# agustinus/emqx

Hardware: AMD Instinct MI355X
Metric: publishes matched/sec (node) at 1M wildcard subs; p99 batch match latency (higher is better)
Workload: dtype u32; 1 GPU; C2: 1M wildcard filters depth<=7, 10M-publish batch per GPU; filters=1000000, publishes_per_gpu=10000000, mode=replicated, parallelism=replicated trie x1, batches split per GPU, batches_in_flight=1

## Files before the change

### emqx_amd/csrc/tm_batch.cpp

```cpp
#include "tm_engine_impl.hpp"

int tm_engine::ensure_slow_scratch(tm_batch* b) {
    int rc;
    if (!b->s_waves) {
        uint32_t w = b->n < 65536 ? 64u : std::min<uint32_t>(TM_SLOW_WAVES_MAX, b->n / 32);
        b->s_waves = w;
    }
    const size_t q = (size_t)b->s_waves * b->s_qcap, o = (size_t)b->s_waves * b->s_ocap;
    if ((rc = b->gen.d_sqpar.reserve(q))) return rc;
    if ((rc = b->gen.d_sqpw.reserve(q))) return rc;
    if ((rc = b->gen.d_sqmeta.reserve(q))) return rc;
    if ((rc = b->gen.d_sqkey.reserve(q))) return rc;
    if ((rc = b->gen.d_sofid.reserve(o))) return rc;
    if ((rc = b->gen.d_sokey.reserve(o))) return rc;
    return TM_OK;
}

void tm_engine::tokenize_range(const TokView& v, uint32_t lo, uint32_t hi, std::vector<uint32_t>& slow_out) const {
    std::vector<TWord> ws;
    for (uint32_t t = lo; t < hi; ++t) {
        const uint8_t* p = v.bytes + v.offs[t];
        const size_t len = v.offs[t + 1] - v.offs[t];
        split_words(p, len, ws);
        uint32_t* out = v.words + v.toff[t];
// ... 867 lines not shown
    HIP_OK(launch_scan(b->scan_args, S, b->dcsr.d_total.p));
    HIP_OK(launch_finalize(b->scan_args, S, checked));
    HIP_OK(hipEventRecord(b->dcsr.evc1.e, S));
    HIP_OK(hipMemcpyAsync(b->dcsr.h_total.p, b->dcsr.d_total.p, 4, hipMemcpyDeviceToHost, S));
    HIP_OK(hipStreamSynchronize(S));
    if (b->dcsr.h_total.p[0] != b->total) {
        snprintf(last_error(), 512, "inconsistent CSR: scanned %u entries, kernel count %llu", b->dcsr.h_total.p[0],
                 (unsigned long long)b->total);
        return TM_EIO;
    }
    float ms = 0;
    (void)hipEventElapsedTime(&ms, b->dcsr.evc0.e, b->dcsr.evc1.e);
    b->st.ms_csr = ms;
    b->dense = true;
    return TM_OK;
}

int tm_engine::check_ctrl(const uint32_t* ctrl, const unsigned long long* stats, uint32_t* err, uint64_t* need,
               uint64_t* staged_out) {
    *err = ctrl[CTRL_ERR];
    uint64_t staged = 0, top = 0;
    for (uint32_t g = 0; g < TICKET_GROUPS; ++g) {
        const uint64_t t = xg_top_read(ctrl, g);
        staged += t;
        top = std::max(top, t);
    }
    *need = top * TICKET_GROUPS;
    if (staged_out) *staged_out = staged;
    const uint64_t nmatch = stats[ST_MATCHES];
    if ((*err & ERR_CSR_RANGE) || staged > result_limit || nmatch > result_limit) {
        snprintf(last_error(), 512, "batch result too large: %llu staged / %llu matched > limit %llu",
                 (unsigned long long)staged, (unsigned long long)nmatch, (unsigned long long)result_limit);
        return TM_EOVERFLOW;
    }
    return TM_OK;
}

int tm_engine::grow_for(tm_batch* b, uint32_t err, uint64_t need, uint64_t staged) {
    if (err & ERR_STAGING) {
        const uint64_t limit = std::min<uint64_t>(MAX_RESULT, result_limit + 1024);
        if (!b->one_region && need + need / 4 + 1024 > limit && staged <= result_limit) b->one_region = true;
        if (b->one_region) need = staged;
        int rc = b->walk.d_sfids.reserve(std::min<uint64_t>(need + need / 4 + 1024, limit));
        if (rc) return rc;
    }
    if (err & ERR_SLOW_SCRATCH) {
        b->s_qcap *= 4;
        b->s_ocap *= 4;
    }
    return TM_OK;
}

void tm_engine::fill_stats(tm_batch* b) {
    float ms_match = 0, ms_total = 0, ms_tok = 0, ms_dd = 0, ms_x = 0;
    (void)hipEventElapsedTime(&ms_match, b->walk.ev0.e, b->walk.ev1.e);
    (void)hipEventElapsedTime(&ms_total, b->walk.ev0.e, b->walk.ev2.e);
    if (b->tok_timed) (void)hipEventElapsedTime(&ms_tok, b->tok.evt.e, b->walk.ev0.e);
    if (b->dedup_timed) (void)hipEventElapsedTime(&ms_dd, b->dd.evd.e, b->tok_timed ? b->tok.evt.e : b->walk.ev0.e);
    if (b->dedup_dev && !b->graphed) (void)hipEventElapsedTime(&ms_x, b->dd.evx0.e, b->dd.evx1.e);
    b->st.ms_tokenize = ms_tok;
    b->st.ms_dedup = ms_dd;
    b->st.ms_expand = ms_x;
    b->st.publishes = b->dedup ? b->n_pub : b->n;
    float ms_q = 0;
    (void)hipEventElapsedTime(&ms_q, b->walk.evq.e,
                              b->dedup_timed ? b->dd.evd.e : b->tok_timed ? b->tok.evt.e : b->walk.ev0.e);
    b->st.ms_queue = ms_q;
    b->st.ms_csr = 0;
    b->st.topics = b->n;
    b->st.visits = b->walk.h_stats[ST_VISITS];
    b->st.hash_hits = b->walk.h_stats[ST_HASH];
    b->st.words = b->walk.h_stats[ST_WORDS];
    b->st.matches = b->walk.h_stats[ST_MATCHES];
    b->st.slow_topics = b->walk.h_stats[ST_SLOW];
    b->st.probes = b->walk.h_stats[ST_PROBES];
    b->st.iterations = b->walk.h_stats[ST_ITERS];
    b->st.overflow_tiles = b->walk.h_ctrl[CTRL_NOVF];
    b->st.ms_match = ms_match;
    b->st.ms_total = ms_total;
    b->total = b->st.matches;
    b->st.delivered = b->dedup_dev ? b->walk.h_stats[ST_DELIVERED] : b->st.matches;
#if TM_PHASE_CYCLES
    fprintf(stderr, "tm_phase_cycles prologue=%llu loop=%llu readback=%llu sort=%llu ms_match=%.4f\n",
            b->h_stats[ST_PHASE + 0], b->h_stats[ST_PHASE + 1], b->h_stats[ST_PHASE + 2], b->h_stats[ST_PHASE + 3],
            ms_match);
#endif
}

int tm_engine::wait(tm_batch* b, bool drained, uint32_t* relaunched) {
    if (!b->launched) return TM_EINVAL;
    const hipStream_t S = st(b);
    if (!b->csr) {
        int rc = launch(b, true);
        if (rc) return rc;
        drained = false;
    }
    for (int attempt = 0;; ++attempt) {
        if (!drained || attempt) {
            if (b->end_recorded) HIP_OK(hipEventSynchronize(b->walk.ev_end.e));
            else HIP_OK(hipStreamSynchronize(S));
        }
        if (attempt && relaunched) ++*relaunched;
        if (b->dedup_dev) {
            b->n = b->walk.h_ctrl[CTRL_NROWS];
            b->scan_args.n = b->n;
        }
        if (b->check_tokens && b->n && b->tok.h_bad.p[1]) {
            snprintf(last_error(), 512, "token batch failed the device check (word offsets or flags)");
            return TM_EINVAL;
        }
        const uint32_t* h_dbg = b->rep->tab.h_dbg.p;
        if (checked && h_dbg[0]) {
            snprintf(last_error(), 512, "bounds check %u failed: index %u bound %u (count %u, extra %u)",
                     h_dbg[0], h_dbg[1], h_dbg[2], h_dbg[3], h_dbg[4]);
            return TM_EIO;
        }
        uint32_t err;
        uint64_t need, staged;
        int rc = check_ctrl(b->walk.h_ctrl, b->walk.h_stats, &err, &need, &staged);
        if (rc) return rc;
        if (!err) break;
        if (attempt >= 6) {
            snprintf(last_error(), 512, "capacity misses did not settle after %d relaunches (err %#x, %llu staged)",
                     attempt, err, (unsigned long long)staged);
            return TM_EOVERFLOW;
        }
        if ((rc = grow_for(b, err, need, staged))) return rc;
        if ((rc = launch(b))) return rc;
    }
    fill_stats(b);
    b->done = true;
    if (b->dedup_dev) b->dtab_dirty = false;
    b->dense = b->dense_enq && !b->oneshot && b->total <= b->dense_cap;
    if (b->dense) {
        float ms = 0;
        (void)hipEventElapsedTime(&ms, b->dcsr.evc0.e, b->dcsr.evc1.e);
        b->st.ms_csr = ms;
    }
    return TM_OK;
}

int tm_engine::result(tm_batch* b, tm_result* out) {
    if (!b->done) return TM_EINVAL;
    int rc;
    if ((rc = ensure_dense(b))) return rc;
    const hipStream_t S = st(b);
    const uint64_t total = b->total;
    if (total > b->dcsr.d_ids.cap) {
        snprintf(last_error(), 512, "inconsistent CSR: kernel count %llu, capacity %zu",
                 (unsigned long long)total, b->dcsr.d_ids.cap);
        return TM_EIO;
    }
    if ((rc = b->dcsr.h_rowoff.reserve((size_t)b->n + 1))) return rc;
    if ((rc = b->dcsr.h_ids.reserve(std::max<uint64_t>(total, 1)))) return rc;
    HIP_OK(hipMemcpyAsync(b->dcsr.h_rowoff.p, b->dcsr.d_rowoff.p, ((size_t)b->n + 1) * 4, hipMemcpyDeviceToHost, S));
    if (total) HIP_OK(hipMemcpyAsync(b->dcsr.h_ids.p, b->dcsr.d_ids.p, total * 4, hipMemcpyDeviceToHost, S));
    HIP_OK(hipStreamSynchronize(S));
    if (b->dcsr.h_rowoff.p[b->n] != total) {
        snprintf(last_error(), 512, "inconsistent CSR: row offsets end at %u, kernel count %llu",
                 b->dcsr.h_rowoff.p[b->n], (unsigned long long)total);
        return TM_EIO;
    }
    out->n_topics = b->n;
    out->n_matches = total;
    out->row_offsets = b->dcsr.h_rowoff.p;
    out->filter_ids = b->dcsr.h_ids.p;
    return TM_OK;
// ... 88 lines not shown
```

### emqx_amd/csrc/tm_kernels.hip

```cpp
#include <algorithm>
#include <cstddef>
#include <cstdlib>
#include "tm_internal.hpp"

namespace etm {

constexpr int TILE = 64;
constexpr int WCAP = 512;
#ifndef TM_WPE384
#define TM_WPE384 4
#endif

constexpr uint32_t M_LVL_SHIFT = 6;
constexpr uint32_t M_LVL_MASK = 0xF;
constexpr uint32_t M_PLUS = 1u << 10;
constexpr uint32_t M_SKIPE = 1u << 11;
constexpr uint32_t M_DSTART = 1u << 12;
static_assert(FAST_MAX_DEPTH <= (int)M_LVL_MASK, "level field too narrow");
constexpr uint32_t M_DISP_SHIFT = 13;
constexpr uint32_t M_DISP_MASK = 0x3F;
constexpr uint32_t Q_FOUND = ~((1u << LSIG_BITS) - 1u);
constexpr uint32_t Q_TAIL = 0xFFFFFFFFu;

__device__ __forceinline__ uint32_t dig_L(uint32_t c) { return (0x4432u >> (4 * c)) & 0xF; }
// ... 89 lines not shown
    if (x.np == 0) { x.pk0 = key; x.pf0 = fl; } else { x.pk1 = key; x.pf1 = fl; }
    x.np++;
}

__device__ __forceinline__ void expand(const Node& s, uint32_t lc, uint32_t d, uint32_t flags,
                                       uint64_t key, uint32_t w_here, uint32_t w_prev, Expand& x) {
    x.ne = 0; x.np = 0;
    if (lc == d) {
        if (!(flags & M_SKIPE) && s.term != NONE) {
            uint64_t k = key;
            if ((w_prev >> WID_BITS) == C_EMPTY && lc - 1 <= FAST_MAX_DEPTH) {
                const int sp = key_shift(lc - 1);
                if (((k >> sp) & 7) == 4) k = (k & ~(7ull << sp)) | (1ull << sp);
            }
            add_e(x, s.term, k);
        }
        if (s.hterm != NONE) add_e(x, s.hterm, put_digit(key, lc, 2));
        return;
    }
    const uint32_t cls = w_here >> WID_BITS, id = w_here & WID_MASK;
    if (s.hterm != NONE) add_e(x, s.hterm, put_digit(key, lc, dig_H(cls)));
    if (id == W_HASH) {
        if (s.flags & NF_HASH) add_p(x, put_digit(key, lc, dig_L(cls)), (lc + 1 == d) ? M_SKIPE : 0u);
    } else if (id != W_UNKNOWN && id != W_PLUS) {
        add_p(x, put_digit(key, lc, dig_L(cls)), 0u);
    }
    if (s.flags & NF_PLUS) add_p(x, put_digit(key, lc, dig_P(cls)), M_PLUS);
}

__device__ __forceinline__ void expand_root(const RootRec& r, bool dollar, uint32_t d, uint32_t w0, Expand& x) {
    x.ne = 0; x.np = 0;
    const uint32_t cls = w0 >> WID_BITS, id = w0 & WID_MASK;
    if (!dollar && r.hterm != NONE) add_e(x, r.hterm, (uint64_t)dig_H(cls) << 61);
    if (id == W_HASH) {
        if (!dollar && (r.flags & NF_HASH)) add_p(x, (uint64_t)dig_L(cls) << 61, (d == 1) ? M_SKIPE : 0u);
    } else if (id != W_UNKNOWN && id != W_PLUS) {
        add_p(x, (uint64_t)dig_L(cls) << 61, dollar ? M_DSTART : 0u);
    }
    if (!dollar && (r.flags & NF_PLUS)) add_p(x, (uint64_t)dig_P(cls) << 61, M_PLUS);
}

template <int QC>
struct alignas(16) TileLds {
    static constexpr int QCAP = QC;
    uint4 q[QC];
    uint32_t words[WCAP];
    uint32_t toff[TILE];
    uint32_t depth[TILE];
    uint32_t cnt[TILE];
    uint32_t list[TILE];
    static constexpr uint32_t STAGE = (QC * 16 + WCAP * 4) / 8;
};

__device__ __forceinline__ uint4 q_pack(uint64_t key, uint32_t meta, uint32_t parent, uint32_t pw) {
    return uint4{(uint32_t)key | meta, (uint32_t)(key >> 32), parent, pw};
}

static_assert(offsetof(TileLds<512>, words) + sizeof(uint32_t) * WCAP == TileLds<512>::STAGE * 8,
              "staging area must be contiguous");
static_assert(offsetof(TileLds<384>, words) + sizeof(uint32_t) * WCAP == TileLds<384>::STAGE * 8,
              "staging area must be contiguous");

__device__ __forceinline__ uint32_t xor_lane32(uint32_t v, uint32_t j) {
    const uint32_t lane = threadIdx.x & 63;
    switch (j) {
    case 1: return (uint32_t)__builtin_amdgcn_mov_dpp((int)v, 0xB1, 0xF, 0xF, false);
    case 2: return (uint32_t)__builtin_amdgcn_mov_dpp((int)v, 0x4E, 0xF, 0xF, false);
    case 4: return (uint32_t)__builtin_amdgcn_mov_dpp(__builtin_amdgcn_mov_dpp((int)v, 0x141, 0xF, 0xF, false), 0x1B, 0xF,
                                                      0xF, false);
    case 8: return (uint32_t)__builtin_amdgcn_mov_dpp((int)v, 0x128, 0xF, 0xF, false);
    case 16: {
        const auto p = __builtin_amdgcn_permlane16_swap(v, v, false, false);
        return (lane & 16) ? p[0] : p[1];
    }
    default: {
        const auto p = __builtin_amdgcn_permlane32_swap(v, v, false, false);
        return (lane & 32) ? p[0] : p[1];
    }
    }
}

__device__ __forceinline__ unsigned long long xor_lane64(unsigned long long v, uint32_t j) {
    return ((unsigned long long)xor_lane32((uint32_t)(v >> 32), j) << 32) | xor_lane32((uint32_t)v, j);
}

enum : int { PH_PROLOGUE = 0, PH_LOOP = 1, PH_READBACK = 2, PH_SORT = 3 };
struct PhaseClk {
#if TM_PHASE_CYCLES
    unsigned long long sum[PHASE_N] = {0, 0, 0, 0}, t0 = 0;
    __device__ __forceinline__ void start() { t0 = __builtin_readcyclecounter(); }
    __device__ __forceinline__ void lap(int p) {
        const unsigned long long now = __builtin_readcyclecounter();
        sum[p] += now - t0;
        t0 = now;
    }
#else
    __device__ __forceinline__ void start() {}
    __device__ __forceinline__ void lap(int) {}
#endif
};

__device__ __forceinline__ uint32_t xor_lane32_bc(uint32_t v, uint32_t j) {
    const int x = (int)v;
    switch (j) {
    case 1: return (uint32_t)__builtin_amdgcn_update_dpp(0, x, 0xB1, 0xF, 0xF, true);
    case 2: return (uint32_t)__builtin_amdgcn_update_dpp(0, x, 0x4E, 0xF, 0xF, true);
    case 4: return (uint32_t)__builtin_amdgcn_update_dpp(0, __builtin_amdgcn_update_dpp(0, x, 0x141, 0xF, 0xF, true),
                                                         0x1B, 0xF, 0xF, true);
    default: return (uint32_t)__builtin_amdgcn_update_dpp(0, x, 0x128, 0xF, 0xF, true);
    }
}

#ifndef TM_TAGGED_SORT
#define TM_TAGGED_SORT 1
#endif
constexpr uint64_t keep_lo_mask(uint32_t W, uint32_t kk, uint32_t j) {
    uint64_t m = 0;
    for (uint32_t l = 0; l < 64; ++l) {
        const uint32_t e = l & (W - 1);
        if (((e & j) == 0) == ((e & kk) == 0)) m |= 1ull << l;
    }
    return m;
}

template <uint32_t W, uint32_t KK, uint32_t J>
__device__ __forceinline__ uint32_t tag_stage(uint32_t k) {
    constexpr uint64_t M = keep_lo_mask(W, KK, J);
    uint32_t lo, hi;
    if constexpr (J >= 16) {
        const auto p = J == 16 ? __builtin_amdgcn_permlane16_swap(k, k, false, false)
                               : __builtin_amdgcn_permlane32_swap(k, k, false, false);
        lo = min(p[0], p[1]);
        hi = max(p[0], p[1]);
    } else {
        const uint32_t other = xor_lane32_bc(k, J);
        lo = min(k, other);
        hi = max(k, other);
    }
    return __builtin_amdgcn_inverse_ballot_w64(M) ? lo : hi;
}
template <uint32_t W, uint32_t KK, uint32_t J>
__device__ __forceinline__ uint32_t tag_merge(uint32_t k) {
    k = tag_stage<W, KK, J>(k);
    if constexpr (J > 1) k = tag_merge<W, KK, J / 2>(k);
    return k;
}
template <uint32_t W, uint32_t KK = 2>
__device__ __forceinline__ uint32_t tag_sort(uint32_t k) {
    k = tag_merge<W, KK, KK / 2>(k);
    if constexpr (KK < W) k = tag_sort<W, KK * 2>(k);
    return k;
}

template <bool CK, class LT>
__device__ __forceinline__ void sort_classes(const MatchArgs& a, LT& L, bool keep, uint32_t c, uint32_t pos,
                                             uint32_t dst, uint32_t free) {
    constexpr uint32_t STAGE = LT::STAGE;
    const uint32_t lane = threadIdx.x;
    const unsigned long long* stg = reinterpret_cast<const unsigned long long*>(L.q);
    if (keep && c == 1) a.sfids[CK_(dst, a.sfids_cap, 40)] = (uint32_t)(stg[CK_(pos, STAGE, 41)] & ~KEY_MASK);
#pragma unroll
    for (uint32_t W = 2; W <= 64; W <<= 1) {
        const bool mine = keep && c > W / 2 && c <= W;
        const uint64_t m = __ballot(mine);
        if (!m) continue;
        const uint32_t nrows = __popcll(m);
        if (mine) L.list[prefix_count(m)] = lane;
        __syncthreads();
        const uint32_t e = lane & (W - 1);
        const uint32_t STEP = 64 / W;
        for (uint32_t g = 0; g < nrows; g += STEP) {
            const uint32_t r = g + lane / W;
            const bool rv = r < nrows;
            const uint32_t owner = rv ? L.list[r] : 0u;
            const uint32_t cr = __shfl(c, owner, 64);
            const uint32_t pr = __shfl(pos, owner, 64);
            const uint32_t dr = __shfl(dst, owner, 64);
            if (TM_TAGGED_SORT && (W >> free) <= 1) {
                const uint32_t* stg32 = reinterpret_cast<const uint32_t*>(L.q);
                uint32_t k32 = 0xFFFFFFFFu;
                if (rv && e < cr) k32 = stg32[2 * CK_(pr + e, STAGE, 42) + 1] | e;
                switch (W) {
                case 2: k32 = tag_sort<2>(k32); break;
                case 4: k32 = tag_sort<4>(k32); break;
                case 8: k32 = tag_sort<8>(k32); break;
                case 16: k32 = tag_sort<16>(k32); break;
                case 32: k32 = tag_sort<32>(k32); break;
                default: k32 = tag_sort<64>(k32); break;
                }
                if (rv && e < cr)
                    a.sfids[CK_((uint64_t)dr + e, a.sfids_cap, 44)] =
                        stg32[2 * CK_(pr + (k32 & (W - 1)), STAGE, 43)] & (uint32_t)~KEY_MASK;
                continue;
            }
            unsigned long long key = ~0ull;
            if (rv && e < cr) key = stg[CK_(pr + e, STAGE, 42)];
#pragma unroll
            for (uint32_t kk = 2; kk <= W; kk <<= 1) {
#pragma unroll
                for (uint32_t j = kk >> 1; j > 0; j >>= 1) {
                    const unsigned long long other = xor_lane64(key, j);
                    const bool up = (e & kk) == 0;
                    const bool lower = (e & j) == 0;
                    const unsigned long long lo = key < other ? key : other;
                    const unsigned long long hi = key < other ? other : key;
                    key = (lower == up) ? lo : hi;
                }
            }
            if (rv && e < cr) a.sfids[CK_((uint64_t)dr + e, a.sfids_cap, 44)] = (uint32_t)(key & ~KEY_MASK);
        }
        __syncthreads();
    }
    {
        const bool mine = keep && c > 64;
        uint64_t m = __ballot(mine);
        while (m) {
            const uint32_t owner = (uint32_t)__builtin_ctzll(m);
            m &= m - 1;
            const uint32_t cr = __shfl(c, owner, 64);
            const uint32_t pr = __shfl(pos, owner, 64);
            const uint32_t dr = __shfl(dst, owner, 64);
            unsigned long long k0 = ~0ull, k1 = ~0ull;
            if (lane < cr) k0 = stg[CK_(pr + lane, STAGE, 45)];
            if (lane + 64 < cr) k1 = stg[CK_(pr + lane + 64, STAGE, 46)];
            uint32_t r0 = 0, r1 = 0;
            for (uint32_t j = 0; j < 64; ++j) {
                const unsigned long long kj = __shfl(k0, j, 64);
                r0 += kj < k0 ? 1u : 0u;
                r1 += kj < k1 ? 1u : 0u;
            }
            for (uint32_t j = 64; j < cr; ++j) {
                const unsigned long long kj = __shfl(k1, j - 64, 64);
                r0 += kj < k0 ? 1u : 0u;
                r1 += kj < k1 ? 1u : 0u;
            }
            if (lane < cr) a.sfids[CK_((uint64_t)dr + r0, a.sfids_cap, 47)] = (uint32_t)(k0 & ~KEY_MASK);
            if (lane + 64 < cr) a.sfids[CK_((uint64_t)dr + r1, a.sfids_cap, 48)] = (uint32_t)(k1 & ~KEY_MASK);
        }
    }
}

#ifndef TM_LOG_U
#define TM_LOG_U 12
#endif
template <bool CK, class LT>
__device__ __forceinline__ void sort_rows_log(const MatchArgs& a, LT& L, bool keep, uint32_t c, uint32_t dst,
                                              unsigned long long* wlog, uint8_t* wlane, uint32_t lcount,
                                              PhaseClk& pc) {
    constexpr uint32_t STAGE = LT::STAGE;
    const uint32_t lane = threadIdx.x;
    unsigned long long* stg = reinterpret_cast<unsigned long long*>(L.q);
    const uint32_t cw = keep ? c : 0u;
    uint32_t incl = cw;
    for (int o = 1; o < 64; o <<= 1) {
        const uint32_t u = __shfl_up(incl, o, 64);
        if (lane >= (uint32_t)o) incl += u;
    }
    const uint32_t pos = incl - cw;
    uint32_t rs = 0;
    while (rs < a.tile_topics) {
        const uint32_t p0 = __builtin_amdgcn_readlane(pos, rs);
        const uint64_t beyond = __ballot(lane >= rs && pos + cw - p0 > STAGE);
        const uint32_t re = beyond ? (uint32_t)__builtin_ctzll(beyond) : a.tile_topics;
        const bool in_chunk = keep && lane >= rs && lane < re;
        L.depth[lane] = in_chunk ? pos - p0 : NONE;
        L.toff[lane] = 0;
        __syncthreads();
        uint32_t kor = 0;
        for (uint32_t k0 = 0; k0 < lcount; k0 += 64 * TM_LOG_U) {
            unsigned long long e[TM_LOG_U];
            uint32_t r[TM_LOG_U];
#pragma unroll
            for (uint32_t u = 0; u < TM_LOG_U; ++u) {
                const uint32_t k = k0 + lane + 64 * u;
                r[u] = 64;
                if (k < lcount) {
                    e[u] = wlog[k];
                    r[u] = wlane[k];
                }
            }
#pragma unroll
            for (uint32_t u = 0; u < TM_LOG_U; ++u) {
                const uint32_t base = r[u] < 64 ? L.depth[r[u]] : NONE;
                if (base == NONE) continue;
                const uint32_t at = base + atomicAdd(&L.toff[r[u]], 1u);
                stg[CK_(at, STAGE, 49)] = e[u];
                kor |= (uint32_t)(e[u] >> 31);
            }
        }
        uint32_t free = 0;
        if (TM_TAGGED_SORT) {
#pragma unroll
            for (uint32_t j = 1; j < 64; j <<= 1) kor |= xor_lane32(kor, j);
            const uint32_t tz = (uint32_t)__builtin_ctz(__builtin_amdgcn_readfirstlane(kor) | 0x200u);
            free = tz ? tz - 1 : 0u;
        }
        __syncthreads();
        pc.lap(PH_READBACK);
        sort_classes<CK, LT>(a, L, in_chunk, c, pos - p0, dst, free);
        __syncthreads();
        pc.lap(PH_SORT);
        rs = re;
    }
}

template <bool CK>
__device__ __forceinline__ void send_to_slow(const MatchArgs& a, bool mine, uint32_t t) {
    const uint64_t m = __ballot(mine);
    uint32_t base = 0;
    if (threadIdx.x == 0 && m) base = atomicAdd(&a.ctrl[CTRL_NOVF], (uint32_t)__popcll(m));
    base = __shfl(base, 0, 64);
    if (mine) {
        const uint32_t slot = base + prefix_count(m);
        if (slot < a.ovf_cap) a.ovf_list[CK_(slot, a.ovf_cap, 12)] = t;
        else atomicOr(&a.ctrl[CTRL_ERR], ERR_OVF_LIST);
    }
}

template <bool CK, bool BIG, bool IN_LDS, class LT>
__device__ __forceinline__ void match_tile(const MatchArgs& a, LT& L, uint32_t t0, uint32_t tend, uint32_t wbase,
                                           uint8_t fl, bool valid, unsigned long long& sV, unsigned long long& sH,
                                           unsigned long long& sW, unsigned long long& sM, unsigned long long& sP,
                                           PhaseClk& pc) {
    const uint32_t lane = threadIdx.x;
    const uint32_t t = t0 + lane;
    const uint32_t* wsrc = IN_LDS ? L.words : a.words;
    const uint32_t wlim = IN_LDS ? (uint32_t)WCAP : a.nwords;
    (void)wbase;

    uint32_t qn = 0;
    const bool active = !(fl & TF_SLOW);
    unsigned long long* const wrows = a.rows + (uint64_t)blockIdx.x * a.tile_topics * a.row_cap;
    const uint32_t lcap = a.tile_topics * a.row_cap;
    uint8_t* const wlane =
        reinterpret_cast<uint8_t*>(a.rows + (uint64_t)a.grid * lcap) + (uint64_t)blockIdx.x * lcap;
    uint32_t lcount = 0;
    uint32_t tV = 0, tH = 0, tW = 0, tP = 0;
    const uint32_t d_me = L.depth[lane];

    {
        Expand x; x.ne = 0; x.np = 0;
        uint32_t w0 = 0;
        if (active && d_me > 0) {
            const bool dollar = fl & TF_DOLLAR;
            tV += 1;
            if (!dollar && (a.root.flags & NF_HASH)) tH += 1;
            tW += d_me;
            w0 = wsrc[CK_(L.toff[lane], wlim, 9)];
            expand_root(a.root, dollar, d_me, w0, x);
        }
        const uint64_t b0 = __ballot(x.np >= 1), b1 = __ballot(x.np >= 2);
        const uint32_t pre = prefix_count(b0) + prefix_count(b1);
        const uint32_t meta = lane | (1u << M_LVL_SHIFT);
        const uint32_t wid = w0 & WID_MASK;
        if (x.np >= 1) L.q[qn + pre] = q_pack(x.pk0, meta | x.pf0, ROOT, (x.pf0 & M_PLUS) ? W_PLUS : wid);
        if (x.np >= 2) L.q[qn + pre + 1] = q_pack(x.pk1, meta | x.pf1, ROOT, (x.pf1 & M_PLUS) ? W_PLUS : wid);
        qn += __popcll(b0) + __popcll(b1);
        const uint64_t mr = __ballot(x.ne != 0);
        if (x.ne) {
            L.cnt[lane] = 1;
            const uint32_t i = prefix_count(mr);
            wrows[i] = (x.ek0 & KEY_MASK) | x.ef0;
            wlane[i] = (uint8_t)lane;
        }
        lcount = (uint32_t)__popcll(mr);
    }

    const uint32_t qd = lane >> 2, qs = lane & 3;
    uint32_t nbk = a.nbuckets, maxp = a.max_probe, rcap = a.row_cap, nrec = BIG ? 0u : a.nslots * 16u;
    Slot* sbase = const_cast<Slot*>(a.slots);
    asm volatile("" : "+s"(nbk), "+s"(maxp), "+s"(rcap), "+s"(nrec), "+s"(sbase));
    uint64_t wbits = IN_LDS ? 0ull : (uint64_t)a.words;
    if constexpr (!IN_LDS) asm volatile("" : "+s"(wbits));
    typedef const __attribute__((address_space(1))) uint32_t* gwords_t;
    typedef uint32_t u32x4_t __attribute__((ext_vector_type(4)));
    typedef const __attribute__((address_space(1))) u32x4_t* gslots_t;
    const auto word_at = [&](uint64_t i) -> uint32_t { return IN_LDS ? L.words[i] : ((gwords_t)wbits)[i]; };
    pc.lap(PH_PROLOGUE);
    while (qn > 0) {
        const uint32_t k = min(qn, 64u);
        const bool has = lane < k;
        qn -= k;
        tP += k + (1u << 20);
        asm volatile("" : "+v"(tP));
        const uint32_t idx = qn + (has ? lane : 0u);
        const uint4 e = L.q[idx];
        const uint32_t meta = e.x & 0x7FFFFFFFu;
        const uint64_t key = ((uint64_t)e.y << 32) | (e.x & 0x80000000u);
        const uint32_t parent = e.z, pw = e.w;
        const uint32_t tl = meta & 63;
        const uint32_t lc = (meta >> M_LVL_SHIFT) & M_LVL_MASK;
        const uint32_t disp = (meta >> M_DISP_SHIFT) & M_DISP_MASK;
        {
            uint32_t hb = home_bucket(parent, pw, nbk) + disp;
            if (hb >= nbk) hb -= nbk;
            L.q[idx].x = hb;
        }
        asm volatile("" : "+s"(sbase), "+s"(nrec));
        const __amdgpu_buffer_rsrc_t rsrc = __builtin_amdgcn_make_buffer_rsrc(sbase, 0, nrec, 0x00020000);
        uint32_t rp[4], rw[4];
        uint4 sl[4];
#pragma unroll
        for (uint32_t r = 0; r < 4; ++r) {
            const uint32_t p = 16 * r + qd;
            const bool v = p < k;
            const uint4 rec = L.q[qn + (v ? p : 0u)];
            rp[r] = v ? rec.z : SLOT_EMPTY;
            rw[r] = rec.w;
            const uint64_t si = CK_((uint64_t)rec.x * BUCKET + qs, a.nslots, 1);
            if (!BIG) {
                sl[r] = ld_b128(rsrc, v ? (uint32_t)si * 16u : 0xFFFFFFF0u);
            } else {
                const u32x4_t g = v ? ((gslots_t)(uint64_t)sbase)[si] : u32x4_t{0u, 0u, 0u, 0u};
                sl[r] = uint4{g[0], g[1], g[2], g[3]};
            }
        }
        __builtin_amdgcn_sched_barrier(0);
        const uint32_t base = L.toff[tl];
        const uint32_t d = L.depth[tl];
        const bool at_end = lc == d;
        const uint32_t w_here = word_at(CK_(base + lc - (at_end ? 1u : 0u), wlim, 11));
        const uint32_t w_prev = word_at(CK_(base + lc - 1, wlim, 10));
#pragma unroll
        for (uint32_t r = 0; r < 4; ++r) {
            const bool m = (sl[r].x & ID_MASK) == rp[r] && (sl[r].y & WID_MASK) == rw[r];
            if (m) {
                L.q[qn + 16 * r + qd].x = sl[r].z;
                L.q[qn + 16 * r + qd].y = sl[r].w;
                L.q[qn + 16 * r + qd].z = Q_FOUND | slot_lsig(sl[r].x, sl[r].y);
            }
        }
        uint32_t qs_now = qs;
        asm volatile("" : "+v"(qs_now));
        if (qs_now == 3) {
#pragma unroll
            for (uint32_t r = 0; r < 4; ++r) L.q[qn + 16 * r + qd].w = sl[r].x == SLOT_EMPTY ? Q_TAIL : rw[r];
        }
        const uint4 res = L.q[idx];
        const bool live = has & (L.cnt[tl] <= rcap);
        const bool found = live & (res.z >= Q_FOUND);
        const bool cont = live & !found & (res.w != Q_TAIL) & (disp < maxp);
        const uint32_t hz = res.x, hw = res.y;
        const uint32_t child = hz & ID_MASK, hterm = hw & ID_MASK;
        const bool n_topic = (hz & B_TOPIC) != 0, n_plus = (hz & B_PLUS) != 0;
        const bool n_hterm = (hw & B_HTERM) != 0, n_hash = (hw & B_HASH) != 0;
        const uint32_t cls = w_here >> WID_BITS, id = w_here & WID_MASK;
        const int sh = key_shift(lc);
        tV += (found & !(meta & M_DSTART)) ? 1u : 0u;
        tH += (found & n_hash) ? 1u : 0u;
        const bool eA0 = found & (at_end ? (!(meta & M_SKIPE) & n_topic) : n_hterm);
        const bool eB0 = found & at_end & n_hterm;
        const uint32_t fA = at_end ? child : hterm;
        const int sp = sh + 3;
        const bool redigit = ((w_prev >> WID_BITS) == C_EMPTY) & (((key >> sp) & 7) == 4);
        const uint64_t kA = key ^ ((uint64_t)(at_end ? (redigit ? 5u : 0u) : dig_H(cls)) << (at_end ? sp : sh));
        const bool lit = (id != W_UNKNOWN) & (id != W_PLUS) & (((res.z >> lsig_pos(id)) & 1u) != 0) &
                         (n_hash | (((hw >> lext_pos(id)) & 1u) != 0));
        const bool pL = found & !at_end & (id == W_HASH ? n_hash : lit);
        const bool pP = found & !at_end & n_plus;
        bool eA = eA0, eB = eB0;
        const bool sL = cont | pL;
        const uint64_t bL = __ballot(sL), bP = __ballot(pP);
        const uint32_t ptot = __popcll(bL) + __popcll(bP);
        if (qn + ptot > (uint32_t)LT::QCAP) break;
        const uint32_t pre = qn + prefix_count(bL) + prefix_count(bP);
        const uint32_t nmeta = tl | ((lc + 1) << M_LVL_SHIFT);
        if (sL) {
            const uint32_t lfl = ((id == W_HASH) & (lc + 1 == d)) ? M_SKIPE : 0u;
            const uint64_t kL = cont ? key : key | ((uint64_t)dig_L(cls) << sh);
            L.q[pre] = q_pack(kL, cont ? meta + (1u << M_DISP_SHIFT) : nmeta | lfl, cont ? parent : child,
                              cont ? pw : id);
        }
        if (pP) L.q[pre + (sL ? 1u : 0u)] = q_pack(key | ((uint64_t)dig_P(cls) << sh), nmeta | M_PLUS, child, W_PLUS);
        qn += ptot;
        {
            uint32_t slot = 0;
            if (eA | eB) slot = atomicAdd(&L.cnt[tl], (eA ? 1u : 0u) + (eB ? 1u : 0u));
            const uint32_t slotB = slot + (eA ? 1u : 0u);
            eA = eA && slot < rcap;
            eB = eB && slotB < rcap;
            const uint64_t mA = __ballot(eA), mB = __ballot(eB);
            const uint32_t nA = (uint32_t)__popcll(mA), nE = nA + (uint32_t)__popcll(mB);
            if (eA) {
                const uint32_t i = lcount + prefix_count(mA);
                wrows[CK_(i, lcap, 13)] = (kA & KEY_MASK) | fA;
                wlane[i] = (uint8_t)tl;
            }
            if (eB) {
                const uint32_t i = lcount + nA + prefix_count(mB);
                wrows[CK_(i, lcap, 14)] = ((key | (2ull << sh)) & KEY_MASK) | hterm;
                wlane[i] = (uint8_t)tl;
            }
            lcount += nE;
        }
    }
    __syncthreads();
    pc.lap(PH_LOOP);

    if (qn > 0) {
        send_to_slow<CK>(a, valid && active, t);
        return;
    }
    sV += tV; sH += tH; sW += tW;
    if (lane == 0) sP += (tP & 0xFFFFFu) | ((unsigned long long)(tP >> 20) << 40);
    const uint32_t c_me = L.cnt[lane];
    const bool row_ovf = valid && active && c_me > a.row_cap;
    send_to_slow<CK>(a, row_ovf, t);
    const bool keep = valid && active && !row_ovf;
    const uint32_t c = keep ? c_me : 0u;
    uint32_t incl = c;
    for (int o = 1; o < 64; o <<= 1) {
        const uint32_t u = __shfl_up(incl, o, 64);
        if (lane >= (uint32_t)o) incl += u;
    }
    const uint32_t tot = __shfl(incl, 63, 64);
    unsigned long long base64 = 0;
    const uint32_t g = (blockIdx.x % TICKET_GROUPS) & a.sgmask;
    if (lane == 0 && tot) base64 = atomicAdd(xg_top(a.xg, g), (unsigned long long)tot);
    base64 = __shfl(base64, 0, 64);
    const bool fits = base64 + tot <= a.rcap;
    base64 += (uint64_t)g * a.rcap;
    const uint32_t base = (uint32_t)base64;
    const uint32_t dst = base + incl - c;
    pc.lap(PH_SORT);
    if (fits) {
        sort_rows_log<CK, LT>(a, L, keep, c, dst, wrows, wlane, lcount, pc);
    } else if (lane == 0) {
        atomicOr(&a.ctrl[CTRL_ERR], ERR_STAGING);
    }
    if (keep) {
        a.count[CK_(t, a.n, 16)] = c_me;
        a.src[CK_(t, a.n, 17)] = dst;
        sM += c_me;
    }
    pc.lap(PH_SORT);
    (void)tend;
}

#ifndef TM_DN_TILES_PER_WAVE
#define TM_DN_TILES_PER_WAVE 4
#endif
constexpr uint32_t DN_TILES_PER_WAVE = TM_DN_TILES_PER_WAVE;

template <bool CK, bool BIG, int QC>
__global__ __launch_bounds__(64) __attribute__((amdgpu_waves_per_eu(QC == 384 ? TM_WPE384 : 3, 8))) void tm_match_tiles(MatchArgs a) {
    __shared__ TileLds<QC> L;
    if (a.d_n) {
        a.n = *a.d_n;
        while (a.tile_topics > 1 && (a.n + a.tile_topics - 1) / a.tile_topics < DN_TILES_PER_WAVE * gridDim.x)
            a.tile_topics >>= 1;
        const uint32_t nt = (a.n + a.tile_topics - 1) / a.tile_topics;
        a.static_rounds = max(1u, nt / (2u * gridDim.x));
    }
    const uint32_t lane = threadIdx.x;
    const uint32_t tt = a.tile_topics;
    const uint32_t ntiles = (a.n + tt - 1) / tt;
    unsigned long long sV = 0, sH = 0, sW = 0, sM = 0, sP = 0;
    PhaseClk pc;

    uint32_t tile = blockIdx.x, round = 0;
    while (tile < ntiles) {
        pc.start();
        uint32_t ticket = 0;
        if (round + 1 >= a.static_rounds && lane == 0)
            ticket = atomicAdd(&a.xg[(blockIdx.x % TICKET_GROUPS) * TICKET_STRIDE], 1u);
        const uint32_t t0 = tile * tt;
        const uint32_t tend = min(t0 + tt, a.n);
        const uint32_t t = t0 + lane;
        const bool valid = lane < tt && t < a.n;
        const uint32_t wbeg = a.toff[CK_(t0, a.n + 1, 2)], wend = a.toff[CK_(tend, a.n + 1, 3)];
        const bool in_lds = (wend - wbeg) <= (uint32_t)WCAP;
        const uint32_t my_off = valid ? a.toff[CK_(t, a.n + 1, 4)] : wend;
        const uint32_t my_end = valid ? a.toff[CK_(t + 1, a.n + 1, 5)] : wend;
        const uint8_t fl = valid ? a.tflags[CK_(t, a.n, 6)] : (uint8_t)TF_SLOW;
        if (in_lds)
            for (uint32_t i = lane; i < wend - wbeg; i += 64) L.words[CK_(i, WCAP, 7)] = a.words[CK_(wbeg + i, a.nwords, 8)];
        L.toff[lane] = in_lds ? my_off - wbeg : my_off;
        L.depth[lane] = my_end - my_off;
        L.cnt[lane] = 0;
        __syncthreads();
        if (in_lds) match_tile<CK, BIG, true>(a, L, t0, tend, wbeg, fl, valid, sV, sH, sW, sM, sP, pc);
        else match_tile<CK, BIG, false>(a, L, t0, tend, wbeg, fl, valid, sV, sH, sW, sM, sP, pc);
        __syncthreads();
        ++round;
        tile = round < a.static_rounds
                   ? blockIdx.x + round * gridDim.x
                   : a.static_rounds * gridDim.x + __builtin_amdgcn_readfirstlane(ticket) * TICKET_GROUPS +
                         blockIdx.x % TICKET_GROUPS;
    }

    for (int o = 32; o > 0; o >>= 1) {
        sV += __shfl_xor(sV, o, 64); sH += __shfl_xor(sH, o, 64);
        sW += __shfl_xor(sW, o, 64); sM += __shfl_xor(sM, o, 64);
        sP += __shfl_xor(sP, o, 64);
    }
    if (lane == 0 && a.wstats) {
        unsigned long long* w = a.wstats + (uint64_t)blockIdx.x * WSTATS;
        w[0] = sV; w[1] = sH; w[2] = sW; w[3] = sM;
        w[4] = sP & ((1ull << 40) - 1); w[5] = sP >> 40;
#if TM_PHASE_CYCLES
        for (uint32_t k = 0; k < PHASE_N; ++k) w[6 + k] = pc.sum[k];
#endif
    } else if (lane == 0) {
        atomicAdd(&a.stats[ST_VISITS], sV); atomicAdd(&a.stats[ST_HASH], sH);
        atomicAdd(&a.stats[ST_WORDS], sW); atomicAdd(&a.stats[ST_MATCHES], sM);
        atomicAdd(&a.stats[ST_PROBES], sP & ((1ull << 40) - 1));
        atomicAdd(&a.stats[ST_ITERS], sP >> 40);
#if TM_PHASE_CYCLES
        for (uint32_t k = 0; k < PHASE_N; ++k) atomicAdd(&a.stats[ST_PHASE + k], pc.sum[k]);
#endif
    }
}

__global__ __launch_bounds__(256) void tm_stats_reduce(const unsigned long long* w, uint32_t waves,
                                                       unsigned long long* stats) {
    constexpr uint32_t NS = 6 + PHASE_N;
    __shared__ unsigned long long sh[4][NS];
    unsigned long long v[NS] = {};
    for (uint32_t i = threadIdx.x; i < waves; i += 256)
#pragma unroll
        for (uint32_t k = 0; k < NS; ++k) v[k] += w[(uint64_t)i * WSTATS + k];
#pragma unroll
    for (uint32_t k = 0; k < NS; ++k) {
        for (int o = 32; o > 0; o >>= 1) v[k] += __shfl_xor(v[k], o, 64);
        if ((threadIdx.x & 63) == 0) sh[threadIdx.x >> 6][k] = v[k];
    }
    __syncthreads();
    if (threadIdx.x < NS) {
        const uint32_t k = threadIdx.x;
        const unsigned long long t = sh[0][k] + sh[1][k] + sh[2][k] + sh[3][k];
        const uint32_t idx[6] = {ST_VISITS, ST_HASH, ST_WORDS, ST_MATCHES, ST_PROBES, ST_ITERS};
        if (t) atomicAdd(&stats[k < 6 ? idx[k] : ST_PHASE + (k - 6)], t);
    }
}


template <bool CK>
__device__ __forceinline__ bool filter_less(const MatchArgs& a, uint32_t x, uint32_t y) {
    if (x == NONE) return false;
    if (y == NONE) return true;
    x = CK_(x, a.nnodes, 20); y = CK_(y, a.nnodes, 21);
    const uint8_t* px = a.fbytes + CK_(a.foff[x], a.nfbytes + 1, 22);
    const uint8_t* py = a.fbytes + CK_(a.foff[y], a.nfbytes + 1, 23);
    const uint32_t lx = a.flen[x], ly = a.flen[y];
    const uint32_t m = min(lx, ly);
    for (uint32_t i = 0; i < m; ++i)
        if (px[i] != py[i]) return px[i] < py[i];
    return lx < ly;
}

template <bool CK>
__device__ void bitonic(const MatchArgs& a, unsigned long long* kp, uint32_t* fp, uint32_t n, bool by_bytes) {
    const uint32_t lane = threadIdx.x;
    for (uint32_t k = 2; k <= n; k <<= 1) {
        for (uint32_t j = k >> 1; j > 0; j >>= 1) {
            for (uint32_t i = lane; i < n; i += 64) {
                const uint32_t ixj = i ^ j;
                if (ixj > i) {
                    const bool up = (i & k) == 0;
                    const bool gt = by_bytes ? filter_less<CK>(a, fp[ixj], fp[i]) : (kp[i] > kp[ixj]);
                    if (gt == up) {
                        const unsigned long long tk = kp[i]; kp[i] = kp[ixj]; kp[ixj] = tk;
                        const uint32_t tf = fp[i]; fp[i] = fp[ixj]; fp[ixj] = tf;
                    }
                }
            }
            __threadfence_block();
            __syncthreads();
        }
    }
}

#ifndef TM_SLOW_SQ
#define TM_SLOW_SQ 512
#endif
constexpr uint32_t SLOW_SQ = TM_SLOW_SQ;
constexpr uint32_t SORT_LDS = SLOW_SQ * 2;
constexpr uint32_t SM_PLUS = 1u << 29;
// ... 2440 lines not shown
```

Measured before the change: 2.550 billion publishes/s.

## Prefetch next tile's offsets, flags and words during current tile's match

Adds a software pipeline in the persistent match kernel: the next tile index is computed early, and its topic offsets/flags are loaded after the walk loop while its word data (up to WCAP) is loaded into registers during the sort phase, then written into LDS at the start of the next iteration. This is meant to hide global-memory latency of the per-tile prologue. Per-lane statistics are also reduced per tile into wave-uniform scalars instead of a final 64-bit shuffle reduction. The prefetch buffer adds registers (WCAP/64 words per lane), which may lower occupancy, and a stale-ticket or tile-ordering issue could arise if next-tile computation changes.

```diff
diff --git a/emqx_amd/csrc/tm_batch.cpp b/emqx_amd/csrc/tm_batch.cpp
--- a/emqx_amd/csrc/tm_batch.cpp
+++ b/emqx_amd/csrc/tm_batch.cpp
@@ -973,7 +973,7 @@
     b->st.delivered = b->dedup_dev ? b->walk.h_stats[ST_DELIVERED] : b->st.matches;
 #if TM_PHASE_CYCLES
     fprintf(stderr, "tm_phase_cycles prologue=%llu loop=%llu readback=%llu sort=%llu ms_match=%.4f\n",
-            b->h_stats[ST_PHASE + 0], b->h_stats[ST_PHASE + 1], b->h_stats[ST_PHASE + 2], b->h_stats[ST_PHASE + 3],
+            b->walk.h_stats[ST_PHASE + 0], b->walk.h_stats[ST_PHASE + 1], b->walk.h_stats[ST_PHASE + 2], b->walk.h_stats[ST_PHASE + 3],
             ms_match);
 #endif
 }
diff --git a/emqx_amd/csrc/tm_kernels.hip b/emqx_amd/csrc/tm_kernels.hip
--- a/emqx_amd/csrc/tm_kernels.hip
+++ b/emqx_amd/csrc/tm_kernels.hip
@@ -195,6 +195,12 @@
 
 __device__ __forceinline__ unsigned long long xor_lane64(unsigned long long v, uint32_t j) {
     return ((unsigned long long)xor_lane32((uint32_t)(v >> 32), j) << 32) | xor_lane32((uint32_t)v, j);
+}
+
+__device__ __forceinline__ uint32_t tile_sum(uint32_t v) {
+#pragma unroll
+    for (uint32_t j = 1; j < 64; j <<= 1) v += xor_lane32(v, j);
+    return __builtin_amdgcn_readfirstlane(v);
 }
 
 enum : int { PH_PROLOGUE = 0, PH_LOOP = 1, PH_READBACK = 2, PH_SORT = 3 };
@@ -353,13 +359,58 @@
     }
 }
 
+#ifndef TM_PREFETCH_NEXT
+#define TM_PREFETCH_NEXT 2
+#endif
+struct TileAhead {
+    uint32_t off, end, fl;
+#if TM_PREFETCH_NEXT >= 2
+    uint32_t w[WCAP / 64];
+#endif
+};
+
+template <bool CK>
+__device__ __forceinline__ void ahead_meta(const MatchArgs& a, uint32_t tile, uint32_t tt, TileAhead& p) {
+    const uint32_t lane = threadIdx.x;
+    const uint32_t t = tile * tt + lane;
+    p.off = 0; p.end = 0; p.fl = TF_SLOW;
+    if (lane < tt && t < a.n) {
+        p.off = a.toff[CK_(t, a.n + 1, 4)];
+        p.end = a.toff[CK_(t + 1, a.n + 1, 5)];
+        p.fl = a.tflags[CK_(t, a.n, 6)];
+    }
+}
+
+__device__ __forceinline__ void ahead_range(const MatchArgs& a, uint32_t tile, uint32_t tt, const TileAhead& p,
+                                            uint32_t& wbeg, uint32_t& wend) {
+    const uint32_t nv = min(tt, a.n - tile * tt);
+    wbeg = __builtin_amdgcn_readlane(p.off, 0);
+    wend = __builtin_amdgcn_readlane(p.end, nv - 1);
+}
+
+template <bool CK>
+__device__ __forceinline__ void ahead_words(const MatchArgs& a, uint32_t tile, uint32_t tt, TileAhead& p) {
+#if TM_PREFETCH_NEXT >= 2
+    const uint32_t lane = threadIdx.x;
+    uint32_t wbeg, wend;
+    ahead_range(a, tile, tt, p, wbeg, wend);
+    const uint32_t nw = wend - wbeg;
+    if (nw > (uint32_t)WCAP) return;
+#pragma unroll
+    for (uint32_t j = 0; j < WCAP / 64; ++j) {
+        const uint32_t i = lane + 64 * j;
+        if (i < nw) p.w[j] = a.words[CK_(wbeg + i, a.nwords, 8)];
+    }
+#endif
+}
+
 #ifndef TM_LOG_U
 #define TM_LOG_U 12
 #endif
-template <bool CK, class LT>
+template <bool CK, class LT, class AW>
 __device__ __forceinline__ void sort_rows_log(const MatchArgs& a, LT& L, bool keep, uint32_t c, uint32_t dst,
                                               unsigned long long* wlog, uint8_t* wlane, uint32_t lcount,
-                                              PhaseClk& pc) {
+                                              PhaseClk& pc, const AW& ah_words) {
     constexpr uint32_t STAGE = LT::STAGE;
     const uint32_t lane = threadIdx.x;
     unsigned long long* stg = reinterpret_cast<unsigned long long*>(L.q);
@@ -410,6 +461,7 @@
         }
         __syncthreads();
         pc.lap(PH_READBACK);
+        if (rs == 0) ah_words();
         sort_classes<CK, LT>(a, L, in_chunk, c, pos - p0, dst, free);
         __syncthreads();
         pc.lap(PH_SORT);
@@ -430,11 +482,11 @@
     }
 }
 
-template <bool CK, bool BIG, bool IN_LDS, class LT>
+template <bool CK, bool BIG, bool IN_LDS, class LT, class AM, class AW>
 __device__ __forceinline__ void match_tile(const MatchArgs& a, LT& L, uint32_t t0, uint32_t tend, uint32_t wbase,
                                            uint8_t fl, bool valid, unsigned long long& sV, unsigned long long& sH,
                                            unsigned long long& sW, unsigned long long& sM, unsigned long long& sP,
-                                           PhaseClk& pc) {
+                                           PhaseClk& pc, const AM& ah_meta, const AW& ah_words) {
     const uint32_t lane = threadIdx.x;
     const uint32_t t = t0 + lane;
     const uint32_t* wsrc = IN_LDS ? L.words : a.words;
@@ -448,7 +500,7 @@
     uint8_t* const wlane =
         reinterpret_cast<uint8_t*>(a.rows + (uint64_t)a.grid * lcap) + (uint64_t)blockIdx.x * lcap;
     uint32_t lcount = 0;
-    uint32_t tV = 0, tH = 0, tW = 0, tP = 0;
+    uint32_t tV = 0, tH = 0, tP = 0;
     const uint32_t d_me = L.depth[lane];
 
     {
@@ -458,7 +510,6 @@
             const bool dollar = fl & TF_DOLLAR;
             tV += 1;
             if (!dollar && (a.root.flags & NF_HASH)) tH += 1;
-            tW += d_me;
             w0 = wsrc[CK_(L.toff[lane], wlim, 9)];
             expand_root(a.root, dollar, d_me, w0, x);
         }
@@ -609,13 +660,19 @@
     }
     __syncthreads();
     pc.lap(PH_LOOP);
+    ah_meta();
 
     if (qn > 0) {
         send_to_slow<CK>(a, valid && active, t);
+        ah_words();
         return;
     }
-    sV += tV; sH += tH; sW += tW;
-    if (lane == 0) sP += (tP & 0xFFFFFu) | ((unsigned long long)(tP >> 20) << 40);
+    sV += tile_sum(tV); sH += tile_sum(tH);
+    sW += tile_sum((active && L.depth[lane] > 0) ? L.depth[lane] : 0u);
+    {
+        const uint32_t p = __builtin_amdgcn_readfirstlane(tP);
+        sP += (p & 0xFFFFFu) | ((unsigned long long)(p >> 20) << 40);
+    }
     const uint32_t c_me = L.cnt[lane];
     const bool row_ovf = valid && active && c_me > a.row_cap;
     send_to_slow<CK>(a, row_ovf, t);
@@ -637,15 +694,16 @@
     const uint32_t dst = base + incl - c;
     pc.lap(PH_SORT);
     if (fits) {
-        sort_rows_log<CK, LT>(a, L, keep, c, dst, wrows, wlane, lcount, pc);
-    } else if (lane == 0) {
-        atomicOr(&a.ctrl[CTRL_ERR], ERR_STAGING);
+        sort_rows_log<CK, LT>(a, L, keep, c, dst, wrows, wlane, lcount, pc, ah_words);
+    } else {
+        if (lane == 0) atomicOr(&a.ctrl[CTRL_ERR], ERR_STAGING);
+        ah_words();
     }
     if (keep) {
         a.count[CK_(t, a.n, 16)] = c_me;
         a.src[CK_(t, a.n, 17)] = dst;
-        sM += c_me;
-    }
+    }
+    sM += __builtin_amdgcn_readfirstlane(tot);
     pc.lap(PH_SORT);
     (void)tend;
 }
@@ -672,6 +730,13 @@
     PhaseClk pc;
 
     uint32_t tile = blockIdx.x, round = 0;
+#if TM_PREFETCH_NEXT
+    TileAhead nx;
+    if (tile < ntiles) {
+        ahead_meta<CK>(a, tile, tt, nx);
+        ahead_words<CK>(a, tile, tt, nx);
+    }
+#endif
     while (tile < ntiles) {
         pc.start();
         uint32_t ticket = 0;
@@ -681,6 +746,26 @@
         const uint32_t tend = min(t0 + tt, a.n);
         const uint32_t t = t0 + lane;
         const bool valid = lane < tt && t < a.n;
+#if TM_PREFETCH_NEXT
+        uint32_t wbeg, wend;
+        ahead_range(a, tile, tt, nx, wbeg, wend);
+        const bool in_lds = (wend - wbeg) <= (uint32_t)WCAP;
+        const uint32_t my_off = valid ? nx.off : wend;
+        const uint32_t my_end = valid ? nx.end : wend;
+        const uint8_t fl = (uint8_t)nx.fl;
+#if TM_PREFETCH_NEXT >= 2
+        if (in_lds) {
+#pragma unroll
+            for (uint32_t j = 0; j < WCAP / 64; ++j) {
+                const uint32_t i = lane + 64 * j;
+                if (i < wend - wbeg) L.words[CK_(i, WCAP, 7)] = nx.w[j];
+            }
+        }
+#else
+        if (in_lds)
+            for (uint32_t i = lane; i < wend - wbeg; i += 64) L.words[CK_(i, WCAP, 7)] = a.words[CK_(wbeg + i, a.nwords, 8)];
+#endif
+#else
         const uint32_t wbeg = a.toff[CK_(t0, a.n + 1, 2)], wend = a.toff[CK_(tend, a.n + 1, 3)];
         const bool in_lds = (wend - wbeg) <= (uint32_t)WCAP;
         const uint32_t my_off = valid ? a.toff[CK_(t, a.n + 1, 4)] : wend;
@@ -688,25 +773,37 @@
         const uint8_t fl = valid ? a.tflags[CK_(t, a.n, 6)] : (uint8_t)TF_SLOW;
         if (in_lds)
             for (uint32_t i = lane; i < wend - wbeg; i += 64) L.words[CK_(i, WCAP, 7)] = a.words[CK_(wbeg + i, a.nwords, 8)];
+#endif
         L.toff[lane] = in_lds ? my_off - wbeg : my_off;
         L.depth[lane] = my_end - my_off;
         L.cnt[lane] = 0;
         __syncthreads();
-        if (in_lds) match_tile<CK, BIG, true>(a, L, t0, tend, wbeg, fl, valid, sV, sH, sW, sM, sP, pc);
-        else match_tile<CK, BIG, false>(a, L, t0, tend, wbeg, fl, valid, sV, sH, sW, sM, sP, pc);
+        uint32_t next = ntiles;
+        const auto next_tile = [&]() -> uint32_t {
+            return round + 1 < a.static_rounds
+                       ? blockIdx.x + (round + 1) * gridDim.x
+                       : a.static_rounds * gridDim.x + __builtin_amdgcn_readfirstlane(ticket) * TICKET_GROUPS +
+                             blockIdx.x % TICKET_GROUPS;
+        };
+#if TM_PREFETCH_NEXT
+        const auto ah_meta = [&] {
+            next = next_tile();
+            if (next < ntiles) ahead_meta<CK>(a, next, tt, nx);
+        };
+        const auto ah_words = [&] {
+            if (next < ntiles) ahead_words<CK>(a, next, tt, nx);
+        };
+#else
+        const auto ah_meta = [&] { next = next_tile(); };
+        const auto ah_words = [] {};
+#endif
+        if (in_lds) match_tile<CK, BIG, true>(a, L, t0, tend, wbeg, fl, valid, sV, sH, sW, sM, sP, pc, ah_meta, ah_words);
+        else match_tile<CK, BIG, false>(a, L, t0, tend, wbeg, fl, valid, sV, sH, sW, sM, sP, pc, ah_meta, ah_words);
         __syncthreads();
         ++round;
-        tile = round < a.static_rounds
-                   ? blockIdx.x + round * gridDim.x
-                   : a.static_rounds * gridDim.x + __builtin_amdgcn_readfirstlane(ticket) * TICKET_GROUPS +
-                         blockIdx.x % TICKET_GROUPS;
-    }
-
-    for (int o = 32; o > 0; o >>= 1) {
-        sV += __shfl_xor(sV, o, 64); sH += __shfl_xor(sH, o, 64);
-        sW += __shfl_xor(sW, o, 64); sM += __shfl_xor(sM, o, 64);
-        sP += __shfl_xor(sP, o, 64);
-    }
+        tile = next;
+    }
+
     if (lane == 0 && a.wstats) {
         unsigned long long* w = a.wstats + (uint64_t)blockIdx.x * WSTATS;
         w[0] = sV; w[1] = sH; w[2] = sW; w[3] = sM;
```

After: 2.579 billion publishes/s (median of 6 runs). +1.1%, better.
